# abhi1kumar/SUP-NeRF

Measured on AMD Instinct MI355X. Metric: rays/sec at 4096 rays x 64 samples (fused render forward), higher is better.
Workload: dtype f32

## Files before the change

### sup-nerf_amd/csrc/snr_mlp16.hip

```cpp
#include <atomic>
#include <type_traits>

#include "snr_mlp16_core.hpp"
#include "snr_host.hpp"

namespace snr {

struct Epi {
    float lo;
    const float* zlds;
    const float* zglb;
    float hi;
};
struct EpiRegs { f32x4 z; };

__device__ __forceinline__ uint32_t spread_nibbles(uint32_t m16) {
    return ((m16 >> 12) & 0xFu) | (((m16 >> 8) & 0xFu) << 8) | (((m16 >> 4) & 0xFu) << 16) | ((m16 & 0xFu) << 24);
}

template <bool LATLDS>
__device__ __forceinline__ EpiRegs epi_load(const Epi& c, int T, int g) {
    EpiRegs e;
    e.z = f32x4{0.f, 0.f, 0.f, 0.f};
    if (LATLDS) e.z = *reinterpret_cast<const f32x4*>(c.zlds + 16 * T + 4 * g);
    else if (c.zglb) e.z = *reinterpret_cast<const f32x4*>(c.zglb + 16 * T + 4 * g);
    return e;
}

template <bool MASKS>
__device__ __forceinline__ void epi_value(const f32x4& acc, f32x4& x, const Epi& c, const EpiRegs& e, int r, uint32_t& m16) {
    float v = acc[r];
    if (MASKS) m16 = __builtin_amdgcn_alignbit(m16, __float_as_uint(0.f - v), 31);
    v = __builtin_amdgcn_fmed3f(v, c.lo, c.hi);
    x[r] = v + e.z[r];
    if (MASKS) asm volatile("" : "+v"(m16));
}

template <int NT>
__device__ __forceinline__ void acc_from_bias(f32x4 (&acc)[16], const float* bias , int g) {
#pragma unroll
    for (int t = 0; t < NT; ++t) acc[t] = *reinterpret_cast<const f32x4*>(bias + 16 * t + 4 * g);
}

template <int NT, int WAVES, bool LATLDS, bool MASKS>
__device__ __forceinline__ void layer_from_acc(f32x4 (&accP)[16], Ring16& ring, float* lds, const float* bias, const Epi& c, int g, const Dma16& dm,
                                               const float* base, bool pre, const f32x4 (&xe)[2], const float* next_first, int next_rows,
                                               uint32_t (&mw)[4], f32x4& a0, f32x4& a1) {
    f32x4 accC[16];
    constexpr int rows_mid = NT * 16;
    constexpr int chunk_floats = rows_mid * KC;
    if (pre) {
        chunk_dma16<WAVES>(dm, base, lds + (ring.cur ^ 1) * WBUF16, lds, rows_mid);
        const float* wb = lds + ring.cur * WBUF16;
        acc_from_bias<NT>(accC, bias, g);
        tile_mma<NT, false>(accC, accP, xe[0], wb + ring.aoff[0], a0, a1, wb + ring.aoff[1]);
        tile_mma<NT, false>(accC, accP, xe[1], wb + ring.aoff[1], a0, a1, nullptr);
        ring_turn(ring);
        first_pair(a0, a1, lds + ring.cur * WBUF16 + ring.aoff[0]);
    } else {
        acc_from_bias<NT>(accC, bias, g);
    }
    constexpr int NG = NT / 2;
    EpiRegs e = epi_load<LATLDS>(c, 0, g);
    f32x4 xa, xb;
    uint32_t m16 = 0u;
#pragma unroll
    for (int r = 3; r >= 0; --r) epi_value<MASKS>(accP[0], xa, c, e, r, m16);
#pragma unroll
    for (int ch = 0; ch < 8; ++ch) {
        const float* src = (ch < 7) ? base + (ch + 1) * chunk_floats : next_first;
        const int rows = (ch < 7) ? rows_mid : next_rows;
        float* const dst = lds + (ring.cur ^ 1) * WBUF16;
        const float* wb = lds + ring.cur * WBUF16;
        const float* const wn = (ch < 7 || NT == 16) ? dst + ring.aoff[0] : nullptr;
        tile_mma<NT, false>(accC, accP, xa, wb + ring.aoff[0], a0, a1, wb + ring.aoff[1], [&](int gi) {
            if (gi == 0) e = epi_load<LATLDS>(c, 2 * ch + 1, g);
            constexpr int PSTEP = (WAVES == 8) ? 2 : 1;
            if (gi % PSTEP == 0 && (gi / PSTEP) * 8 * WAVES < rows) chunk_piece16<WAVES>(dm, src, dst, lds, rows, gi / PSTEP);
#pragma unroll
            for (int k = (gi * 4) / NG; k < ((gi + 1) * 4) / NG; ++k) epi_value<MASKS>(accP[2 * ch + 1], xb, c, e, 3 - k, m16);
        });
        if (ch & 1) { mw[ch >> 1] = m16; m16 = 0u; }
        if (ch == 7) {
            tile_mma<NT, true>(accC, accP, xb, wb + ring.aoff[1], a0, a1, wn, NoBetween(), RingTurn());
        } else {
            tile_mma<NT, false>(accC, accP, xb, wb + ring.aoff[1], a0, a1, wn, [&](int gi) {
                if (gi == 0) e = epi_load<LATLDS>(c, 2 * ch + 2, g);
#pragma unroll
                for (int k = (gi * 4) / NG; k < ((gi + 1) * 4) / NG; ++k) epi_value<MASKS>(accP[2 * ch + 2], xa, c, e, 3 - k, m16);
            }, RingTurn());
        }
        ring.cur ^= 1;
    }
}

__device__ __forceinline__ void store_masks16x4(uint4* __restrict__ dst , const uint32_t (&mw)[4], int wave, int lane) {
    const int n = lane & 15, g = lane >> 4;
    uint32_t w[4];
#pragma unroll
    for (int i = 0; i < 4; ++i) {
        const uint32_t mine = spread_nibbles(mw[i]) << (4 * (g >> 1));
        w[i] = mine | (uint32_t)__shfl_xor((int)mine, 32, 64);
    }
    if (g < 2) dst[16 * (wave & 1) + n + 32 * g] = make_uint4(w[0], w[1], w[2], w[3]);
}

#ifdef SNR_STAMPS
#define SNR16_STAMP(i) do { if (io.sigmas && lane == 0) { unsigned long long t_; asm volatile("s_memtime %0\n\ts_waitcnt lgkmcnt(0)" : "=s"(t_) :: "memory"); \
        reinterpret_cast<unsigned long long*>(io.sigmas)[(tile_wg * WAVES + wave) * 8 + (i)] = t_; } } while (0)
#define SNR16_STAMP_HWID(i) do { if (io.sigmas && lane == 0) { unsigned a_, b_; asm volatile("s_getreg_b32 %0, hwreg(HW_REG_HW_ID)\n\ts_getreg_b32 %1, hwreg(HW_REG_XCC_ID)" : "=s"(a_), "=s"(b_)); \
        reinterpret_cast<unsigned long long*>(io.sigmas)[(tile_wg * WAVES + wave) * 8 + (i)] = (unsigned long long)a_ | ((unsigned long long)b_ << 32); } } while (0)
#else
#define SNR16_STAMP(i) do {} while (0)
#define SNR16_STAMP_HWID(i) do {} while (0)
#endif

template <int MODE> struct PointSrc { using T = RayGeom; };
template <> struct PointSrc<MODE_LATTICE> { using T = snr_lattice; };
template <> struct PointSrc<MODE_BRICKS> { using T = BrickSrc; };

template <int MODE, int WAVES, bool LATLDS, bool MASKS>
__global__ void __launch_bounds__(WAVES * 64, 2)
decoder_fwd16_kernel(DecoderIO io, Layout L, Lds16 lo, const float* __restrict__ xyz, const float* __restrict__ viewdir, typename PointSrc<MODE>::T gm,
                     float* __restrict__ out_rgb, float* __restrict__ out_depth, float* __restrict__ out_acc) {
    extern __shared__ __attribute__((aligned(16))) float lds[];
    constexpr int WGP = WAVES * 16;
    constexpr bool DENS = MODE >= 2;
    const int tid = threadIdx.x, lane = tid & 63, wave = tid >> 6, n = lane & 15, g = lane >> 4;
    const long long tile_wg = blockIdx.x;
    const long long gp_raw = tile_wg * WGP + wave * 16 + n;
    const bool live = gp_raw < io.n_points;
    const long long gp = live ? gp_raw : io.n_points - 1;
    const long long tile32 = tile_wg * (WAVES / 2) + (wave >> 1);
    const bool tile_live = tile32 * 32 < io.n_points;
    const int sb = io.sb, tb = io.tb;
    const int n_relu = n_relu_layers(sb, tb);
    SNR16_STAMP(0);
    __builtin_amdgcn_s_setprio(3);
    float px, py, pz, dx, dy, dz, zc = 0.f;
    long long b_obj = 0, b_dst = 0;
    bool b_keep = false;
    if constexpr (MODE == 0) {
        px = xyz[gp * 3]; py = xyz[gp * 3 + 1]; pz = xyz[gp * 3 + 2];
        dx = viewdir[gp * 3]; dy = viewdir[gp * 3 + 1]; dz = viewdir[gp * 3 + 2];
    } else if constexpr (MODE == 1) {
        const PointId id = point_id(gm, tile_wg, WGP, wave * 16 + n, live);
        const SamplePoint sp = make_sample(gm, id.ray, id.s, id.obj);
        px = sp.x; py = sp.y; pz = sp.z; dx = sp.dx; dy = sp.dy; dz = sp.dz; zc = sp.zc;
    } else if constexpr (MODE == 2) {
        px = xyz[gp * 3]; py = xyz[gp * 3 + 1]; pz = xyz[gp * 3 + 2];
        dx = dy = dz = 0.f;
    } else if constexpr (MODE == 3) {
        const long long obj = gp / io.points_per_obj;
        const unsigned v = (unsigned)(gp - obj * io.points_per_obj), nyz = (unsigned)(gm.n[1] * gm.n[2]);
        const unsigned i = v / nyz, jk = v - i * nyz, j = jk / (unsigned)gm.n[2], k = jk - j * (unsigned)gm.n[2];
        px = gm.lo[0] + gm.h[0] * (float)i; py = gm.lo[1] + gm.h[1] * (float)j; pz = gm.lo[2] + gm.h[2] * (float)k;
        dx = dy = dz = 0.f;
    } else {
        const int* bk = gm.bricks + ((tile_wg * WGP) >> 9) * 4;
        const int nb0 = (gm.lat.n[0] + 7) >> 3, nb1 = (gm.lat.n[1] + 7) >> 3, nb2 = (gm.lat.n[2] + 7) >> 3;
        const bool ok = bk[0] >= 0 && bk[0] < gm.n_objects && bk[1] >= 0 && bk[1] < nb0 && bk[2] >= 0 && bk[2] < nb1 && bk[3] >= 0 && bk[3] < nb2;
        b_obj = ok ? bk[0] : 0;
        const unsigned l = (unsigned)(gp & 511);
        const unsigned i = 8u * (unsigned)(ok ? bk[1] : 0) + (l >> 6), j = 8u * (unsigned)(ok ? bk[2] : 0) + ((l >> 3) & 7u),
                       k = 8u * (unsigned)(ok ? bk[3] : 0) + (l & 7u);
        px = gm.lat.lo[0] + gm.lat.h[0] * (float)i; py = gm.lat.lo[1] + gm.lat.h[1] * (float)j; pz = gm.lat.lo[2] + gm.lat.h[2] * (float)k;
        dx = dy = dz = 0.f;
        b_keep = ok && i < (unsigned)gm.lat.n[0] && j < (unsigned)gm.lat.n[1] && k < (unsigned)gm.lat.n[2];
        b_dst = b_obj * ((long long)gm.lat.n[0] * gm.lat.n[1] * gm.lat.n[2]) + ((long long)i * gm.lat.n[1] + j) * gm.lat.n[2] + k;
    }
    const float* bias = lds + lo.bias;
    const float* heads = bias + L.n_mfma_layers * 256;
    const float* zero = lds + lo.zero;
    const float* lat_lane = io.latent + (MODE == 4 ? b_obj : gp / io.points_per_obj) * (long long)L.n_lat * 256;
    const float* lat_wg = io.latent + (MODE == 4 ? b_obj : (tile_wg * WGP) / io.points_per_obj) * (long long)L.n_lat * 256;

    Ring16 ring;
    ring.cur = 0;
    Dma16 dm;
    dm.voff = lane * 16u + 4096u;
    dm.lds0 = __builtin_amdgcn_readfirstlane((unsigned)(size_t)(__attribute__((address_space(3))) float*)lds);
    dm.wave = __builtin_amdgcn_readfirstlane(wave);
    {
        const int sw = (n >> 1) & 7;
        ring.aoff[0] = n * KC + (((0 + g) ^ sw) << 2);
        ring.aoff[1] = n * KC + (((4 + g) ^ sw) << 2);
    }
    constexpr long long C256 = 256 * KC;
    const int li_encshape = sb + 1, li_view = sb + 2, li_last = sb + tb + 2;
    const float* const stream = io.packed + L.fwd;
    auto layer_base = [&](int li) { return stream + 2 * C256 + (long long)(li - 1) * 8 * C256 + (li > li_view ? C256 : 0); };
    auto layer_first = [&](int li) { return layer_base(li) + (li == li_view ? 8 * C256 : 0); };
    f32x4 xin[4], xd[2];
    {
        chunk_dma16<WAVES>(dm, stream, lds, lds, 256);
        for (int r = dm.wave; r < L.n_mfma_layers + 3; r += WAVES) row_dma16(dm, io.packed + L.bias + r * 256, lds + lo.bias + r * 256, lds);
        if (LATLDS)
            for (int r = dm.wave; r < L.n_lat; r += WAVES) row_dma16(dm, lat_wg + r * 256, lds + lo.lat + r * 256, lds);
        if (tid < 64) *reinterpret_cast<f32x4*>(lds + lo.zero + 4 * tid) = f32x4{0.f, 0.f, 0.f, 0.f};
        float* sc = lds + lo.scratch + wave * PE_WAVE16 + n * PE_ROW;
#pragma unroll 1
        for (int i = 0; i < 8; i += 2) {
            const int q = 8 * g + i;
            if (q < 3 * XYZ_FREQ) {
                f32x2 sn, cs;
                pe_sincos2(f32x2{ldexpf(pick3(px, py, pz, q % 3), q / 3), ldexpf(pick3(px, py, pz, (q + 1) % 3), (q + 1) / 3)}, &sn, &cs);
                sc[3 + q] = sn[0]; sc[3 + 3 * XYZ_FREQ + q] = cs[0];
                sc[4 + q] = sn[1]; sc[4 + 3 * XYZ_FREQ + q] = cs[1];
            }
        }
        if constexpr (!DENS) {
            const int q = 3 * g;
            f32x2 sn, cs;
            pe_sincos2(f32x2{ldexpf(pick3(dx, dy, dz, q % 3), q / 3), ldexpf(pick3(dx, dy, dz, (q + 1) % 3), (q + 1) / 3)}, &sn, &cs);
            sc[64 + 3 + q] = sn[0]; sc[64 + 3 + 3 * DIR_FREQ + q] = cs[0];
            sc[64 + 4 + q] = sn[1]; sc[64 + 4 + 3 * DIR_FREQ + q] = cs[1];
            float s1, c1;
            pe_sincos(ldexpf(pick3(dx, dy, dz, (q + 2) % 3), (q + 2) / 3), &s1, &c1);
            sc[64 + 5 + q] = s1; sc[64 + 5 + 3 * DIR_FREQ + q] = c1;
        }
        if (g == 0) {
            sc[0] = px; sc[1] = py; sc[2] = pz; sc[63] = 0.f;
            if constexpr (!DENS) {
                sc[64] = dx; sc[65] = dy; sc[66] = dz;
#pragma unroll
                for (int f = D_DIR; f < 32; ++f) sc[64 + f] = 0.f;
            }
        }
        asm volatile("s_waitcnt vmcnt(0)" ::: "memory");
        __syncthreads();
#pragma unroll
        for (int T = 0; T < 4; ++T)
#pragma unroll
            for (int r = 0; r < 4; ++r) xin[T][r] = sc[16 * T + 4 * g + r];
#pragma unroll
        for (int T = 0; T < 2; ++T)
#pragma unroll
            for (int r = 0; r < 4; ++r) xd[T][r] = DENS ? 0.f : sc[64 + 16 * T + 4 * g + r];
        if (WAVES == 4) __syncthreads();
    }

    __builtin_amdgcn_s_setprio(0);
    SNR16_STAMP(1);
    f32x4 accP[16];
    f32x4 a0, a1;
    {
        f32x4 accC[16];
        acc_from_bias<16>(accC, bias, g);
#pragma unroll
        for (int ch = 0; ch < 2; ++ch) {
            chunk_dma16<WAVES>(dm, ch == 0 ? stream + C256 : layer_first(1), lds + (ring.cur ^ 1) * WBUF16, lds, 256);
            const float* wb = lds + ring.cur * WBUF16;
            first_pair(a0, a1, wb + ring.aoff[0]);
            tile_mma<16, false>(accC, accP, xin[2 * ch], wb + ring.aoff[0], a0, a1, wb + ring.aoff[1]);
            if (ch == 1) tile_mma<16, true>(accC, accP, xin[2 * ch + 1], wb + ring.aoff[1], a0, a1, nullptr);
            else tile_mma<16, false>(accC, accP, xin[2 * ch + 1], wb + ring.aoff[1], a0, a1, nullptr);
            ring_turn(ring);
        }
        first_pair(a0, a1, lds + ring.cur * WBUF16 + ring.aoff[0]);
    }

    SNR16_STAMP(2);
    uint32_t mw[4] = {0u, 0u, 0u, 0u};
    float o_sigma = 0.f;
    float pos_inf = __builtin_inff();
    asm volatile("" : "+v"(pos_inf));
    auto epi_of = [&](int lp) {
        const int la = latent_after(lp, sb, tb);
        Epi c;
        c.lo = (lp != li_encshape) ? 0.f : -__builtin_inff();
        c.zlds = (la >= 0) ? lds + lo.lat + la * 256 : zero;
        c.zglb = (la >= 0) ? lat_lane + la * 256 : nullptr;
        c.hi = pos_inf;
        return c;
    };
    auto after_layer_input = [&](int lp) {
        if (MASKS && lp != li_encshape && tile_live) store_masks16x4(io.masks + (tile32 * n_relu + relu_slot(lp, sb)) * 64, mw, wave, lane);
    };
    const int li_stop = DENS ? li_encshape : li_last;
#pragma unroll 1
    for (int li = 1; li <= li_stop; ++li) {
        const int lp = li - 1;
        const Epi c = epi_of(lp);
        if (!DENS && li == li_view) {
            SNR16_STAMP(3);
            float s = 0.f;
#pragma unroll
            for (int T = 0; T < 16; ++T) {
                const f32x4 ws = *reinterpret_cast<const f32x4*>(heads + 16 * T + 4 * g);
#pragma unroll
                for (int r = 0; r < 4; ++r) s = fmaf(ws[r], accP[T][r], s);
            }
            s += __shfl_xor(s, 16, 64);
            s += __shfl_xor(s, 32, 64);
            const float pre = s + heads[L.sigma_b - L.sigma_w];
            o_sigma = pre > 20.f ? pre : log1pf(expf(pre));
        }
        const bool end = DENS && li == li_stop;
        layer_from_acc<16, WAVES, LATLDS, MASKS>(accP, ring, lds, bias + li * 256, c, g, dm, layer_base(li), !DENS && li == li_view, xd,
                                                       end ? nullptr : layer_first(li + 1), end ? 0 : (li == li_last) ? 128 : 256, mw, a0, a1);
        after_layer_input(lp);
    }
    if constexpr (DENS) {
        float s = 0.f;
#pragma unroll
        for (int T = 0; T < 16; ++T) {
            const f32x4 ws = *reinterpret_cast<const f32x4*>(heads + 16 * T + 4 * g);
#pragma unroll
            for (int r = 0; r < 4; ++r) s = fmaf(ws[r], accP[T][r], s);
        }
        s += __shfl_xor(s, 16, 64);
        s += __shfl_xor(s, 32, 64);
        const float pre = s + heads[L.sigma_b - L.sigma_w];
        o_sigma = pre > 20.f ? pre : log1pf(expf(pre));
        if constexpr (MODE == 4) {
            if (b_keep && g == 0) io.sigmas[b_dst] = o_sigma;
        } else {
            if (live && g == 0) io.sigmas[gp] = o_sigma;
        }
        return;
    }
    SNR16_STAMP(4);
    {
        const Epi c = epi_of(li_last);
        layer_from_acc<8, WAVES, LATLDS, MASKS>(accP, ring, lds, bias + (li_last + 1) * 256, c, g, dm, layer_base(li_last + 1), false, xd, nullptr, 0, mw, a0, a1);
        after_layer_input(li_last);
    }

    SNR16_STAMP(5);
    __builtin_amdgcn_s_setprio(3);
    float o_r, o_g, o_b;
    {
        const float* w2 = heads + (L.rgb2_w - L.sigma_w);
        float pr = 0.f, pg = 0.f, pb = 0.f;
        uint32_t m16 = 0u, mr[4] = {0u, 0u, 0u, 0u};
#pragma unroll
        for (int T = 0; T < 8; ++T) {
            const f32x4 wr = *reinterpret_cast<const f32x4*>(w2 + 16 * T + 4 * g);
            const f32x4 wg = *reinterpret_cast<const f32x4*>(w2 + 128 + 16 * T + 4 * g);
            const f32x4 wb = *reinterpret_cast<const f32x4*>(w2 + 256 + 16 * T + 4 * g);
            f32x4 xv;
#pragma unroll
            for (int r = 3; r >= 0; --r) {
                float v = accP[T][r];
                m16 = __builtin_amdgcn_alignbit(m16, __float_as_uint(0.f - v), 31);
                v = fmaxf(v, 0.f);
                xv[r] = v;
            }
#pragma unroll
            for (int r = 0; r < 4; ++r) { pr = fmaf(wr[r], xv[r], pr); pg = fmaf(wg[r], xv[r], pg); pb = fmaf(wb[r], xv[r], pb); }
            if ((T & 3) == 3) { mr[T >> 2] = m16; m16 = 0u; }
        }
        if (MASKS && tile_live) store_masks16x4(io.masks + (tile32 * n_relu + (n_relu - 1)) * 64, mr, wave, lane);
        pr += __shfl_xor(pr, 16, 64); pr += __shfl_xor(pr, 32, 64);
        pg += __shfl_xor(pg, 16, 64); pg += __shfl_xor(pg, 32, 64);
        pb += __shfl_xor(pb, 16, 64); pb += __shfl_xor(pb, 32, 64);
        const float* b2 = heads + (L.rgb2_b - L.sigma_w);
        o_r = pr + b2[0]; o_g = pg + b2[1]; o_b = pb + b2[2];
    }

    SNR16_STAMP_HWID(6);
#ifndef SNR_STAMPS
    if (live && g == 0 && io.sigmas) io.sigmas[gp] = o_sigma;
#endif
    if (live && g == 0) {
        if (io.rgbs) { io.rgbs[gp * 3] = o_r; io.rgbs[gp * 3 + 1] = o_g; io.rgbs[gp * 3 + 2] = o_b; }
    }
    if constexpr (MODE == 1) {
        float* comp = lds + lo.comp;
        if (g == 0) {
            float* c = comp + (wave * 16 + n) * COMP_STRIDE;
            c[0] = o_sigma; c[1] = o_r; c[2] = o_g; c[3] = o_b; c[4] = zc;
        }
        __syncthreads();
        composite_rays_fwd<WGP, WAVES>(comp, gm.S, gm.flags & SNR_WHITE_BKGD, gm.n_rays, tile_wg, wave, lane, out_rgb, out_depth, out_acc);
    }
    SNR16_STAMP(7);
}

}

using namespace snr;


template <int MODE, int WAVES, bool LATLDS, bool MASKS>
static int launch16(const DecoderIO& io, const Layout& L, const Lds16& lo, const float* xyz, const float* viewdir, const typename PointSrc<MODE>::T& g,
                    float* rgb, float* depth, float* acc, hipStream_t st) {
    auto kern = decoder_fwd16_kernel<MODE, WAVES, LATLDS, MASKS>;
    static std::atomic<uint64_t> granted{0};
    int dev = 0;
    if (hipGetDevice(&dev) != hipSuccess) return SNR_E_LAUNCH;
    const uint64_t bit = dev < 64 ? (uint64_t)1 << dev : 0;
    if (!(granted.load(std::memory_order_acquire) & bit)) {
        if (hipFuncSetAttribute(reinterpret_cast<const void*>(kern), hipFuncAttributeMaxDynamicSharedMemorySize, 160 * 1024) != hipSuccess) return SNR_E_LAUNCH;
        granted.fetch_or(bit, std::memory_order_release);
    }
    const unsigned grid = (unsigned)((io.n_points + WAVES * 16 - 1) / (WAVES * 16));
    kern<<<grid, WAVES * 64, (size_t)lo.total * 4, st>>>(io, L, lo, xyz, viewdir, g, rgb, depth, acc);
    return snr_check_launch_();
}

struct Shape16 { int waves; bool latlds; Lds16 lo; };
static Shape16 launch_shape16(int mode, const DecoderIO& io, const Layout& L, int S) {
    auto with = [&](int waves) {
        Shape16 s;
        s.waves = waves;
        s.latlds = (io.points_per_obj % (waves * 16)) == 0 && L.n_lat <= LDS_LAT_ROWS;
        s.lo = make_lds16(waves, L.n_mfma_layers, s.latlds ? L.n_lat : LDS_LAT_ROWS + 1);
        return s;
    };
    const Shape16 four = with(4);
    const bool fits = four.lo.total * 4 <= 80 * 1024 && (mode != MODE_RENDER || (S <= 64 && 64 % S == 0));
    return fits ? four : with(8);
}

template <int MODE, int WAVES>
static int launch16_flags(const Shape16& s, const DecoderIO& io, const Layout& L, const float* xyz, const float* viewdir, const typename PointSrc<MODE>::T& src,
                          float* rgb, float* depth, float* acc, hipStream_t st) {
    auto go = [&](auto latlds, auto masks) {
        return launch16<MODE, WAVES, decltype(latlds)::value, decltype(masks)::value>(io, L, s.lo, xyz, viewdir, src, rgb, depth, acc, st);
    };
    constexpr std::true_type Y{};
    constexpr std::false_type N{};
    const bool ll = s.latlds, mk = io.masks != nullptr;
    if constexpr (MODE == MODE_POINTS || MODE == MODE_RENDER) return ll ? (mk ? go(Y, Y) : go(Y, N)) : (mk ? go(N, Y) : go(N, N));
    else if constexpr (MODE == MODE_DENSITY) return mk ? (ll ? go(Y, Y) : go(N, Y)) : (ll ? go(Y, N) : go(N, N));
    else return ll ? go(Y, N) : go(N, N);
}

int snr_fp32_fwd16_launch_(int mode, const DecoderIO& io, const Layout& L, const float* xyz, const float* viewdir, const RayGeom& g, float* rgb,
                           float* depth, float* acc, void* stream_) {
    hipStream_t st = (hipStream_t)stream_;
    if (io.act) return SNR_E_UNSUPPORTED;
    const Shape16 s = launch_shape16(mode, io, L, g.S);
    if (s.waves == 4) return mode == MODE_POINTS ? launch16_flags<MODE_POINTS, 4>(s, io, L, xyz, viewdir, g, rgb, depth, acc, st)
                                                 : launch16_flags<MODE_RENDER, 4>(s, io, L, xyz, viewdir, g, rgb, depth, acc, st);
    return mode == MODE_POINTS ? launch16_flags<MODE_POINTS, 8>(s, io, L, xyz, viewdir, g, rgb, depth, acc, st)
                               : launch16_flags<MODE_RENDER, 8>(s, io, L, xyz, viewdir, g, rgb, depth, acc, st);
}

template <int MODE>
static int density_launch(const DecoderIO& io, const float* xyz, const typename PointSrc<MODE>::T& src, void* stream_) {
    const Layout L = make_layout(io.sb, io.tb);
    const Shape16 s = launch_shape16(MODE, io, L, 0);
    hipStream_t st = (hipStream_t)stream_;
    return s.waves == 4 ? launch16_flags<MODE, 4>(s, io, L, xyz, nullptr, src, nullptr, nullptr, nullptr, st)
                        : launch16_flags<MODE, 8>(s, io, L, xyz, nullptr, src, nullptr, nullptr, nullptr, st);
}

int snr_density_points_launch_(const DecoderIO& io, const float* xyz, void* stream_) { return density_launch<MODE_DENSITY>(io, xyz, RayGeom{}, stream_); }

int snr_density_bricks_launch_(const DecoderIO& io_, const BrickSrc& src, long long n_bricks, void* stream_) {
    constexpr long long CHUNK = 1 << 20;
    for (long long off = 0; off < n_bricks; off += CHUNK) {
        const long long n = n_bricks - off < CHUNK ? n_bricks - off : CHUNK;
        DecoderIO io = io_;
        io.n_points = n * 512;
        const int rc = density_launch<MODE_BRICKS>(io, nullptr, BrickSrc{src.lat, src.bricks + off * 4, src.n_objects}, stream_);
        if (rc != SNR_OK) return rc;
    }
    return SNR_OK;
}

int snr_density_lattice_launch_(const DecoderIO& io, const snr_lattice& lattice, void* stream_) { return density_launch<MODE_LATTICE>(io, nullptr, lattice, stream_); }
```

### sup-nerf_amd/csrc/snr_mlp16_core.hpp

```cpp
#pragma once
#include "snr_mlp_core.hpp"

namespace snr {

constexpr int PE_WAVE16 = 16 * PE_ROW;
constexpr int WBUF16 = 256 * KC;

struct Lds16 { int ring1, scratch, comp, bias, lat, zero, total; };
inline Lds16 make_lds16(int waves, int n_mfma_layers, int n_lat) {
    Lds16 o;
    o.ring1 = WBUF16;
    int p = 2 * WBUF16;
    if (waves == 8) { o.scratch = p; p += 8 * PE_WAVE16; o.comp = p; p += 128 * COMP_STRIDE; }
    else { o.scratch = o.ring1; o.comp = 0; }
    p = (p + 3) & ~3;
    o.bias = p; p += (n_mfma_layers + 3) * 256;
    o.lat = p; p += (n_lat <= LDS_LAT_ROWS ? n_lat : 0) * 256;
    o.zero = p; p += 256;
    o.total = p;
    return o;
}

template <int K>
__device__ __forceinline__ void dma_piece_imm(unsigned voff, const void* sbase, unsigned m0v) {
    asm volatile("s_mov_b32 m0, %2\n\ts_nop 0\n\tglobal_load_lds_dwordx4 %0, %1 offset:%3" :: "v"(voff), "s"(sbase), "s"(m0v), "n"(1024 * K - 4096) : "memory");
}
__device__ __forceinline__ void dma_piece(int k, unsigned voff, const void* sbase, unsigned m0v) {
    switch (k) {
        case 0: dma_piece_imm<0>(voff, sbase, m0v); break;
        case 1: dma_piece_imm<1>(voff, sbase, m0v); break;
        case 2: dma_piece_imm<2>(voff, sbase, m0v); break;
        case 3: dma_piece_imm<3>(voff, sbase, m0v); break;
        case 4: dma_piece_imm<4>(voff, sbase, m0v); break;
        case 5: dma_piece_imm<5>(voff, sbase, m0v); break;
        case 6: dma_piece_imm<6>(voff, sbase, m0v); break;
        default: dma_piece_imm<7>(voff, sbase, m0v); break;
    }
}
struct Dma16 {
    unsigned voff;
    unsigned lds0;
    int wave;
};
template <int WAVES>
__device__ __forceinline__ void chunk_piece16(const Dma16& d, const float* __restrict__ g, const float* lds_dst, const float* lds_base, int rows, int i) {
    const unsigned sl = (unsigned)(rows * 128 / WAVES) * (unsigned)d.wave;
    const char* sbase = reinterpret_cast<const char*>(g) + sl;
    const unsigned m0v = __builtin_amdgcn_readfirstlane(d.lds0 + (unsigned)((lds_dst - lds_base) * 4) + sl + 4096u);
    dma_piece(i, d.voff, sbase, m0v);
}
template <int WAVES>
__device__ __forceinline__ void chunk_dma16(const Dma16& d, const float* __restrict__ g, const float* lds_dst, const float* lds_base, int rows) {
#pragma unroll
    for (int i = 0; i < 32 / WAVES; ++i)
        if (i * 8 * WAVES < rows) chunk_piece16<WAVES>(d, g, lds_dst, lds_base, rows, i);
}
__device__ __forceinline__ void row_dma16(const Dma16& d, const float* __restrict__ g, const float* lds_dst, const float* lds_base) {
    const unsigned m0v = __builtin_amdgcn_readfirstlane(d.lds0 + (unsigned)((lds_dst - lds_base) * 4) + 4096u);
    dma_piece_imm<0>(d.voff, g, m0v);
}

struct PointId { long long ray, obj; int s; };
__device__ __forceinline__ PointId point_id(const RayGeom& g, long long tile_wg, int wgp, int pl, bool live) {
    const int ls = 31 - __builtin_clz((unsigned)g.S);
    const long long ray0 = tile_wg * (long long)(wgp >> ls);
    const long long obj0 = ray0 / g.rays_per_obj;
    const long long rem0 = ray0 - obj0 * g.rays_per_obj;
    const int dr = pl >> ls;
    const long long r = rem0 + dr;
    PointId p;
    p.ray = ray0 + dr;
    p.s = pl & (g.S - 1);
    p.obj = obj0 + (g.rays_per_obj >= wgp ? (long long)(r >= g.rays_per_obj) : (long long)((unsigned)r / (unsigned)g.rays_per_obj));
    if (!live) { p.ray = g.n_rays - 1; p.s = g.S - 1; p.obj = (g.n_rays - 1) / g.rays_per_obj; }
    return p;
}

struct Ring16 {
    int cur;
    int aoff[2];
};

#define SNR16_WAIT_LDS() __builtin_amdgcn_s_waitcnt(0xc07f)

struct NoBetween { __device__ __forceinline__ void operator()(int) const {} };
struct NoTurn { __device__ __forceinline__ void operator()() const {} };
constexpr int TM_LAST = 1, TM_ZERO = 2;
template <int NT, int FLAGS, class Between = NoBetween, class Turn = NoTurn, int NA = 16, int ND = 16>
__device__ __forceinline__ void tile_mma(f32x4 (&accC)[NA], f32x4 (&accD)[ND], const f32x4& x, const float* wrow ,
                                         f32x4& a0, f32x4& a1, const float* wnext, Between&& between = NoBetween(), Turn&& turn = Turn()) {
    constexpr bool LAST = FLAGS & TM_LAST, ZERO = FLAGS & TM_ZERO;
    const f32x4 zero4 = {0.f, 0.f, 0.f, 0.f};
#pragma unroll
    for (int t = 0; t < NT; t += 2) {
        SNR16_WAIT_LDS();
        f32x4 n0 = a0, n1 = a1;
        if (t + 2 < NT) {
            n0 = *reinterpret_cast<const f32x4*>(wrow + (t + 2) * 16 * KC);
            n1 = *reinterpret_cast<const f32x4*>(wrow + (t + 3) * 16 * KC);
        } else {
            turn();
            if (wnext) {
                n0 = *reinterpret_cast<const f32x4*>(wnext);
                n1 = *reinterpret_cast<const f32x4*>(wnext + 16 * KC);
            }
        }
        __builtin_amdgcn_sched_barrier(0);
#pragma unroll
        for (int r = 0; r < 4; ++r) {
            if (LAST && r == 3) {
                accD[t] = __builtin_amdgcn_mfma_f32_16x16x4f32(a0[r], x[r], accC[t], 0, 0, 0);
                accD[t + 1] = __builtin_amdgcn_mfma_f32_16x16x4f32(a1[r], x[r], accC[t + 1], 0, 0, 0);
            } else {
                accC[t] = __builtin_amdgcn_mfma_f32_16x16x4f32(a0[r], x[r], (ZERO && r == 0) ? zero4 : accC[t], 0, 0, 0);
                accC[t + 1] = __builtin_amdgcn_mfma_f32_16x16x4f32(a1[r], x[r], (ZERO && r == 0) ? zero4 : accC[t + 1], 0, 0, 0);
            }
        }
        between(t / 2);
        __builtin_amdgcn_sched_barrier(0);
        a0 = n0; a1 = n1;
    }
}

__device__ __forceinline__ void first_pair(f32x4& a0, f32x4& a1, const float* wrow) {
    a0 = *reinterpret_cast<const f32x4*>(wrow);
    a1 = *reinterpret_cast<const f32x4*>(wrow + 16 * KC);
}

__device__ __forceinline__ void ring_turn(Ring16& p) {
    asm volatile("s_waitcnt vmcnt(0)" ::: "memory");
    __syncthreads();
    p.cur ^= 1;
}

struct RingTurn {
    __device__ __forceinline__ void operator()() const {
        asm volatile("s_waitcnt vmcnt(0)" ::: "memory");
        __syncthreads();
    }
};


}
```

Baseline: 2.502 million.

## Split view-direction layer work across waves when a workgroup holds one ray

When every point in a workgroup belongs to the same ray (S equals the workgroup point count), the view-direction input contribution is identical for all points. Each wave now computes only its own slice of output rows for that contribution, folds it into the bias in LDS, and then the full layer reloads the updated bias. This is meant to remove redundant MFMA work on the view-direction pre-pass, at the cost of extra LDS writes, an offset prefetch pointer for the next layer, and writes into a bias buffer the code treats as const.

```diff
diff --git a/sup-nerf_amd/csrc/snr_mlp16.hip b/sup-nerf_amd/csrc/snr_mlp16.hip
--- a/sup-nerf_amd/csrc/snr_mlp16.hip
+++ b/sup-nerf_amd/csrc/snr_mlp16.hip
@@ -42,20 +42,38 @@
     for (int t = 0; t < NT; ++t) acc[t] = *reinterpret_cast<const f32x4*>(bias + 16 * t + 4 * g);
 }
 
-template <int NT, int WAVES, bool LATLDS, bool MASKS>
+template <int NT, int WAVES, bool LATLDS, bool MASKS, bool RAY = false>
 __device__ __forceinline__ void layer_from_acc(f32x4 (&accP)[16], Ring16& ring, float* lds, const float* bias, const Epi& c, int g, const Dma16& dm,
                                                const float* base, bool pre, const f32x4 (&xe)[2], const float* next_first, int next_rows,
-                                               uint32_t (&mw)[4], f32x4& a0, f32x4& a1) {
+                                               uint32_t (&mw)[4], f32x4& a0, f32x4& a1, bool ray = false, int next_off = 0) {
     f32x4 accC[16];
     constexpr int rows_mid = NT * 16;
     constexpr int chunk_floats = rows_mid * KC;
     if (pre) {
         chunk_dma16<WAVES>(dm, base, lds + (ring.cur ^ 1) * WBUF16, lds, rows_mid);
-        const float* wb = lds + ring.cur * WBUF16;
-        acc_from_bias<NT>(accC, bias, g);
-        tile_mma<NT, false>(accC, accP, xe[0], wb + ring.aoff[0], a0, a1, wb + ring.aoff[1]);
-        tile_mma<NT, false>(accC, accP, xe[1], wb + ring.aoff[1], a0, a1, nullptr);
+        const bool once = RAY && NT == 16 && ray;
+        if (once) {
+            constexpr int NTW = 16 / WAVES;
+            const float* wb = lds + ring.cur * WBUF16 + own_rows16<WAVES>(dm);
+            float* own = const_cast<float*>(bias) + dm.wave * (NTW * 16) + 4 * g;
+            f32x4 accS[NTW];
+#pragma unroll
+            for (int t = 0; t < NTW; ++t) accS[t] = *reinterpret_cast<const f32x4*>(own + 16 * t);
+            tile_mma<NTW, 0, NoBetween, NoTurn, NTW>(accS, accP, xe[0], wb + ring.aoff[0], a0, a1, wb + ring.aoff[1]);
+            tile_mma<NTW, 0, NoBetween, NoTurn, NTW>(accS, accP, xe[1], wb + ring.aoff[1], a0, a1, nullptr);
+            if ((threadIdx.x & 15) == 0) {
+#pragma unroll
+                for (int t = 0; t < NTW; ++t) *reinterpret_cast<f32x4*>(own + 16 * t) = accS[t];
+            }
+            SNR16_WAIT_LDS();
+        } else {
+            const float* wb = lds + ring.cur * WBUF16;
+            acc_from_bias<NT>(accC, bias, g);
+            tile_mma<NT, false>(accC, accP, xe[0], wb + ring.aoff[0], a0, a1, wb + ring.aoff[1]);
+            tile_mma<NT, false>(accC, accP, xe[1], wb + ring.aoff[1], a0, a1, nullptr);
+        }
         ring_turn(ring);
+        if (once) acc_from_bias<NT>(accC, bias, g);
         first_pair(a0, a1, lds + ring.cur * WBUF16 + ring.aoff[0]);
     } else {
         acc_from_bias<NT>(accC, bias, g);
@@ -72,7 +90,7 @@
         const int rows = (ch < 7) ? rows_mid : next_rows;
         float* const dst = lds + (ring.cur ^ 1) * WBUF16;
         const float* wb = lds + ring.cur * WBUF16;
-        const float* const wn = (ch < 7 || NT == 16) ? dst + ring.aoff[0] : nullptr;
+        const float* const wn = (ch < 7 || NT == 16) ? dst + ring.aoff[0] + ((RAY && ch == 7) ? next_off : 0) : nullptr;
         tile_mma<NT, false>(accC, accP, xa, wb + ring.aoff[0], a0, a1, wb + ring.aoff[1], [&](int gi) {
             if (gi == 0) e = epi_load<LATLDS>(c, 2 * ch + 1, g);
             constexpr int PSTEP = (WAVES == 8) ? 2 : 1;
@@ -278,6 +296,8 @@
         if (MASKS && lp != li_encshape && tile_live) store_masks16x4(io.masks + (tile32 * n_relu + relu_slot(lp, sb)) * 64, mw, wave, lane);
     };
     const int li_stop = DENS ? li_encshape : li_last;
+    bool one_ray = false;
+    if constexpr (MODE == 1) one_ray = gm.S == WGP;
 #pragma unroll 1
     for (int li = 1; li <= li_stop; ++li) {
         const int lp = li - 1;
@@ -297,6 +317,10 @@
             o_sigma = pre > 20.f ? pre : log1pf(expf(pre));
         }
         const bool end = DENS && li == li_stop;
+        if constexpr (MODE == 1)
+            layer_from_acc<16, WAVES, LATLDS, MASKS, true>(accP, ring, lds, bias + li * 256, c, g, dm, layer_base(li), li == li_view, xd, layer_first(li + 1),
+                                                                 (li == li_last) ? 128 : 256, mw, a0, a1, one_ray, (one_ray && li + 1 == li_view) ? own_rows16<WAVES>(dm) : 0);
+        else
         layer_from_acc<16, WAVES, LATLDS, MASKS>(accP, ring, lds, bias + li * 256, c, g, dm, layer_base(li), !DENS && li == li_view, xd,
                                                        end ? nullptr : layer_first(li + 1), end ? 0 : (li == li_last) ? 128 : 256, mw, a0, a1);
         after_layer_input(lp);
diff --git a/sup-nerf_amd/csrc/snr_mlp16_core.hpp b/sup-nerf_amd/csrc/snr_mlp16_core.hpp
--- a/sup-nerf_amd/csrc/snr_mlp16_core.hpp
+++ b/sup-nerf_amd/csrc/snr_mlp16_core.hpp
@@ -76,6 +76,9 @@
     return p;
 }
 
+template <int WAVES>
+__device__ __forceinline__ int own_rows16(const Dma16& d) { return d.wave * ((16 / WAVES) * 16 * KC); }
+
 struct Ring16 {
     int cur;
     int aoff[2];
```

After: 2.529 million, median of 6. +1.1%, better.
